# dylkot/cNMF

Measured on NVIDIA H100. Metric: NMF restarts/sec on NxG counts, K-sweep x100 seeds, 1/2/4/8 H100 vs sklearn CPU, higher is better.
Workload: dtype f32 (2-pass split-fp16 tensor-core products of group-normalised factors x exact integer counts, fp32 accumulate)

## Files before the change

cnmf_b200/csrc/gemm_tf32x3.cu:

```cuda
#include <cuda.h>
#include <cuda_runtime.h>
#include <cstdint>
#include <cstdio>
#include <algorithm>
#include <map>
#include <mutex>
#include <tuple>

#include "common.cuh"
#include "gemm.h"

namespace cnmf {

namespace {

constexpr int BM = 128;
constexpr int BN = 128;
constexpr int BK = 32;
constexpr int NUM_THREADS = 384;
constexpr long long WAIT_TIMEOUT_CYCLES = 4000000000LL;

template <int STAGES, bool BEXACT>
struct SmemLayout {
  static constexpr int A_BYTES = BM * BK * 4;
  static constexpr int B_BYTES = BN * BK * 4;
  static constexpr int STAGE_BYTES = 2 * A_BYTES + (BEXACT ? 1 : 2) * B_BYTES;
  static constexpr int BAR_OFFSET = STAGES * STAGE_BYTES;
  static constexpr int TOTAL = BAR_OFFSET + 2 * STAGES * 8;
  static constexpr int DYN_BYTES = TOTAL + 1024;
  static_assert(DYN_BYTES <= 227 * 1024, "pipeline stages do not fit the shared memory of an SM");
};

__device__ __forceinline__ void mbar_init(uint32_t bar, uint32_t count) {
  asm volatile("mbarrier.init.shared::cta.b64 [%0], %1;" ::"r"(bar), "r"(count) : "memory");
}
__device__ __forceinline__ void mbar_arrive_expect_tx(uint32_t bar, uint32_t bytes) {
  asm volatile("mbarrier.arrive.expect_tx.shared::cta.b64 _, [%0], %1;" ::"r"(bar), "r"(bytes) : "memory");
}
__device__ __forceinline__ void mbar_arrive(uint32_t bar) {
  asm volatile("mbarrier.arrive.shared::cta.b64 _, [%0];" ::"r"(bar) : "memory");
}
__device__ __forceinline__ bool mbar_try_wait(uint32_t bar, uint32_t parity) {
  uint32_t ok;
  asm volatile(
      "{\n\t.reg .pred p;\n\t"
      "mbarrier.try_wait.parity.shared::cta.b64 p, [%1], %2;\n\t"
      "selp.u32 %0, 1, 0, p;\n\t}"
      : "=r"(ok)
      : "r"(bar), "r"(parity)
      : "memory");
  return ok != 0;
}
__device__ __forceinline__ void mbar_wait(uint32_t bar, uint32_t parity) {
  if (mbar_try_wait(bar, parity)) return;
  const long long t0 = clock64();
  while (!mbar_try_wait(bar, parity)) {
    if (clock64() - t0 > WAIT_TIMEOUT_CYCLES) __trap();
  }
}
__device__ __forceinline__ void tma_load_2d(uint32_t dst, const CUtensorMap* map, uint32_t bar, int c0, int c1) {
  asm volatile(
      "cp.async.bulk.tensor.2d.shared::cluster.global.mbarrier::complete_tx::bytes [%0], [%1, {%3, %4}], [%2];"
      ::"r"(dst), "l"(reinterpret_cast<uint64_t>(map)), "r"(bar), "r"(c0), "r"(c1)
      : "memory");
}

__device__ __forceinline__ uint64_t make_smem_desc(uint32_t smem_addr) {
  uint64_t d = 0;
  d |= static_cast<uint64_t>((smem_addr & 0x3FFFFu) >> 4);
  d |= static_cast<uint64_t>(1) << 16;
  d |= static_cast<uint64_t>(1024 >> 4) << 32;
  d |= static_cast<uint64_t>(1) << 62;
  return d;
}

__device__ __forceinline__ void named_bar_sync(uint32_t id, uint32_t count) {
  asm volatile("bar.sync %0, %1;" ::"r"(id), "r"(count) : "memory");
}
__device__ __forceinline__ void named_bar_arrive(uint32_t id, uint32_t count) {
  asm volatile("bar.arrive %0, %1;" ::"r"(id), "r"(count) : "memory");
}

__device__ __forceinline__ void wgmma_fence() { asm volatile("wgmma.fence.sync.aligned;" ::: "memory"); }
__device__ __forceinline__ void wgmma_commit() { asm volatile("wgmma.commit_group.sync.aligned;" ::: "memory"); }
template <int N>
__device__ __forceinline__ void wgmma_wait() { asm volatile("wgmma.wait_group.sync.aligned %0;" ::"n"(N) : "memory"); }

template <bool F16>
__device__ __forceinline__ void wgmma_m64n128(float (&d)[64], uint64_t adesc, uint64_t bdesc, uint32_t acc) {
  if constexpr (F16) {
    asm volatile(
      "{\n\t.reg .pred p;\n\t"
      "setp.ne.b32 p, %66, 0;\n\t"
      "wgmma.mma_async.sync.aligned.m64n128k16.f32.f16.f16 {"
      "%0, %1, %2, %3, %4, %5, %6, %7, %8, %9, %10, %11, %12, %13, %14, %15, "
      "%16, %17, %18, %19, %20, %21, %22, %23, %24, %25, %26, %27, %28, %29, %30, %31, "
      "%32, %33, %34, %35, %36, %37, %38, %39, %40, %41, %42, %43, %44, %45, %46, %47, "
      "%48, %49, %50, %51, %52, %53, %54, %55, %56, %57, %58, %59, %60, %61, %62, %63 "
      "}, %64, %65, p, 1, 1, 0, 0;\n\t}"
      : "+f"(d[0]), "+f"(d[1]), "+f"(d[2]), "+f"(d[3]), "+f"(d[4]), "+f"(d[5]), "+f"(d[6]), "+f"(d[7]),
        "+f"(d[8]), "+f"(d[9]), "+f"(d[10]), "+f"(d[11]), "+f"(d[12]), "+f"(d[13]), "+f"(d[14]), "+f"(d[15]),
        "+f"(d[16]), "+f"(d[17]), "+f"(d[18]), "+f"(d[19]), "+f"(d[20]), "+f"(d[21]), "+f"(d[22]), "+f"(d[23]),
        "+f"(d[24]), "+f"(d[25]), "+f"(d[26]), "+f"(d[27]), "+f"(d[28]), "+f"(d[29]), "+f"(d[30]), "+f"(d[31]),
        "+f"(d[32]), "+f"(d[33]), "+f"(d[34]), "+f"(d[35]), "+f"(d[36]), "+f"(d[37]), "+f"(d[38]), "+f"(d[39]),
        "+f"(d[40]), "+f"(d[41]), "+f"(d[42]), "+f"(d[43]), "+f"(d[44]), "+f"(d[45]), "+f"(d[46]), "+f"(d[47]),
        "+f"(d[48]), "+f"(d[49]), "+f"(d[50]), "+f"(d[51]), "+f"(d[52]), "+f"(d[53]), "+f"(d[54]), "+f"(d[55]),
        "+f"(d[56]), "+f"(d[57]), "+f"(d[58]), "+f"(d[59]), "+f"(d[60]), "+f"(d[61]), "+f"(d[62]), "+f"(d[63])
      : "l"(adesc), "l"(bdesc), "r"(acc));
  } else {
    asm volatile(
      "{\n\t.reg .pred p;\n\t"
      "setp.ne.b32 p, %66, 0;\n\t"
      "wgmma.mma_async.sync.aligned.m64n128k8.f32.tf32.tf32 {"
      "%0, %1, %2, %3, %4, %5, %6, %7, %8, %9, %10, %11, %12, %13, %14, %15, "
      "%16, %17, %18, %19, %20, %21, %22, %23, %24, %25, %26, %27, %28, %29, %30, %31, "
      "%32, %33, %34, %35, %36, %37, %38, %39, %40, %41, %42, %43, %44, %45, %46, %47, "
      "%48, %49, %50, %51, %52, %53, %54, %55, %56, %57, %58, %59, %60, %61, %62, %63 "
      "}, %64, %65, p, 1, 1;\n\t}"
      : "+f"(d[0]), "+f"(d[1]), "+f"(d[2]), "+f"(d[3]), "+f"(d[4]), "+f"(d[5]), "+f"(d[6]), "+f"(d[7]),
        "+f"(d[8]), "+f"(d[9]), "+f"(d[10]), "+f"(d[11]), "+f"(d[12]), "+f"(d[13]), "+f"(d[14]), "+f"(d[15]),
        "+f"(d[16]), "+f"(d[17]), "+f"(d[18]), "+f"(d[19]), "+f"(d[20]), "+f"(d[21]), "+f"(d[22]), "+f"(d[23]),
        "+f"(d[24]), "+f"(d[25]), "+f"(d[26]), "+f"(d[27]), "+f"(d[28]), "+f"(d[29]), "+f"(d[30]), "+f"(d[31]),
        "+f"(d[32]), "+f"(d[33]), "+f"(d[34]), "+f"(d[35]), "+f"(d[36]), "+f"(d[37]), "+f"(d[38]), "+f"(d[39]),
        "+f"(d[40]), "+f"(d[41]), "+f"(d[42]), "+f"(d[43]), "+f"(d[44]), "+f"(d[45]), "+f"(d[46]), "+f"(d[47]),
        "+f"(d[48]), "+f"(d[49]), "+f"(d[50]), "+f"(d[51]), "+f"(d[52]), "+f"(d[53]), "+f"(d[54]), "+f"(d[55]),
        "+f"(d[56]), "+f"(d[57]), "+f"(d[58]), "+f"(d[59]), "+f"(d[60]), "+f"(d[61]), "+f"(d[62]), "+f"(d[63])
      : "l"(adesc), "l"(bdesc), "r"(acc));
  }
}

struct TileOrder {
  int m_tiles, n_tiles, group, group_n;
};

__host__ __device__ __forceinline__ void decode_item(int w, const TileOrder& o, int& mt, int& nt, int& z) {
  const int per_slice = o.m_tiles * o.n_tiles;
  z = w / per_slice;
  int r = w - z * per_slice;
  const int q_tiles = o.group_n ? o.n_tiles : o.m_tiles;
  const int p_tiles = o.group_n ? o.m_tiles : o.n_tiles;
  const int g0 = r / (o.group * p_tiles) * o.group;
  r -= g0 * p_tiles;
  const int gq = q_tiles - g0 < o.group ? q_tiles - g0 : o.group;
  const int p = r / gq, q = g0 + r % gq;
  mt = o.group_n ? p : q;
  nt = o.group_n ? q : p;
}

template <int STAGES, bool BEXACT, bool F16>
__device__ __forceinline__ void
gemm_body(const CUtensorMap& tmA_hi, const CUtensorMap& tmA_lo, const CUtensorMap& tmB_hi, const CUtensorMap& tmB_lo,
          float* __restrict__ C, int M, int ldc, long long c_split_stride,
          const TileOrder& ord, int splits, int total_kb, int kb_per_split, int chain_kb,
          const float* __restrict__ out_scale, const float* __restrict__ a_tile_scale, int a_tiles, int a_gshift) {
  static_assert(!F16 || BEXACT, "the fp16 path exists for exact integer B operands only");
  constexpr int BKE = F16 ? 2 * BK : BK;
  constexpr int KSTEP_BYTES = 32;
  using L = SmemLayout<STAGES, BEXACT>;
  extern __shared__ uint8_t smem_raw[];
  const uint32_t smem_base = (smem_u32(smem_raw) + 1023u) & ~1023u;

  const uint32_t bar_base = smem_base + L::BAR_OFFSET;
  auto full_bar = [&](int s) { return bar_base + 8u * s; };
  auto empty_bar = [&](int s) { return bar_base + 8u * (STAGES + s); };

  const int wg = threadIdx.x >> 7;
  const int warp = (threadIdx.x >> 5) & 3;
  const int lane = threadIdx.x & 31;

  if (threadIdx.x == 0) {
    for (int s = 0; s < STAGES; ++s) {
      mbar_init(full_bar(s), 1);
      mbar_init(empty_bar(s), 8);
    }
    asm volatile("fence.mbarrier_init.release.cluster;" ::: "memory");
  }
  __syncthreads();

  const int items = ord.m_tiles * ord.n_tiles * splits;

  if (wg == 0) {
    if (threadIdx.x == 0) {
      int stage = 0;
      uint32_t phase = 0;
      constexpr uint32_t stage_tx = static_cast<uint32_t>(L::STAGE_BYTES);
      for (int w = blockIdx.x; w < items; w += gridDim.x) {
        int mt, nt, z;
        decode_item(w, ord, mt, nt, z);
        const int kb0 = z * kb_per_split;
        const int kb1 = min(total_kb, kb0 + kb_per_split);
        for (int kb = kb0; kb < kb1; ++kb) {
          mbar_wait(empty_bar(stage), phase ^ 1u);
          const uint32_t st = smem_base + stage * L::STAGE_BYTES;
          mbar_arrive_expect_tx(full_bar(stage), stage_tx);
          tma_load_2d(st, &tmA_hi, full_bar(stage), kb * BKE, mt * BM);
          tma_load_2d(st + L::A_BYTES, &tmA_lo, full_bar(stage), kb * BKE, mt * BM);
          tma_load_2d(st + 2 * L::A_BYTES, &tmB_hi, full_bar(stage), kb * BKE, nt * BN);
          if constexpr (!BEXACT) tma_load_2d(st + 2 * L::A_BYTES + L::B_BYTES, &tmB_lo, full_bar(stage), kb * BKE, nt * BN);
          if (++stage == STAGES) { stage = 0; phase ^= 1u; }
        }
      }
    }
  } else {
    constexpr uint32_t TURN_BAR = 1, TURN_THREADS = 256;
    const int cw = wg - 1;
    const uint32_t a_off = static_cast<uint32_t>(cw * 64 * 128);
    if (cw == 1) named_bar_arrive(TURN_BAR, TURN_THREADS);
    int stage = 0;
    uint32_t phase = 0;
    for (int w = blockIdx.x; w < items; w += gridDim.x) {
      int mt, nt, z;
      decode_item(w, ord, mt, nt, z);
      const int kb0 = z * kb_per_split;
      const int kb1 = min(total_kb, kb0 + kb_per_split);
      const int row0 = mt * BM + cw * 64 + warp * 16 + (lane >> 2);
      float acc[64];
#pragma unroll
      for (int i = 0; i < 64; ++i) acc[i] = 0.f;
      const float* sc_row0 = (F16 && a_tile_scale && row0 < M) ? a_tile_scale + static_cast<long long>(row0) * a_tiles : nullptr;
      const float* sc_row1 = (F16 && a_tile_scale && row0 + 8 < M) ? a_tile_scale + static_cast<long long>(row0 + 8) * a_tiles : nullptr;
      for (int c0 = kb0; c0 < kb1; c0 += chain_kb) {
        const int c1 = min(kb1, c0 + chain_kb);
        float d[64];
        int prev = -1;
        for (int kb = c0; kb < c1; ++kb) {
          mbar_wait(full_bar(stage), phase);
          named_bar_sync(TURN_BAR + cw, TURN_THREADS);
          const uint32_t st = smem_base + stage * L::STAGE_BYTES;
          const uint64_t a_hi = make_smem_desc(st + a_off);
          const uint64_t a_lo = make_smem_desc(st + L::A_BYTES + a_off);
          const uint64_t b_hi = make_smem_desc(st + 2 * L::A_BYTES);
          const uint64_t b_lo = make_smem_desc(st + 2 * L::A_BYTES + L::B_BYTES);
          wgmma_fence();
#pragma unroll
          for (int k = 0; k < BK * 4 / KSTEP_BYTES; ++k) {
            const uint64_t koff = static_cast<uint64_t>((k * KSTEP_BYTES) >> 4);
            const uint32_t acc0 = (kb > c0 || k > 0) ? 1u : 0u;
            wgmma_m64n128<F16>(d, a_lo + koff, b_hi + koff, acc0);
            if constexpr (!BEXACT) wgmma_m64n128<F16>(d, a_hi + koff, b_lo + koff, 1u);
            wgmma_m64n128<F16>(d, a_hi + koff, b_hi + koff, 1u);
          }
          wgmma_commit();
          named_bar_arrive(TURN_BAR + (cw ^ 1), TURN_THREADS);
          if (prev >= 0) {
            wgmma_wait<1>();
            if (lane == 0) mbar_arrive(empty_bar(prev));
          }
          prev = stage;
          if (++stage == STAGES) { stage = 0; phase ^= 1u; }
        }
        wgmma_wait<0>();
        if (lane == 0) mbar_arrive(empty_bar(prev));
        if constexpr (F16) {
          const float s0 = sc_row0 ? sc_row0[c0 >> a_gshift] : 1.f;
          const float s1 = sc_row1 ? sc_row1[c0 >> a_gshift] : 1.f;
#pragma unroll
          for (int i = 0; i < 64; i += 4) {
            acc[i] = fmaf(d[i], s0, acc[i]);
            acc[i + 1] = fmaf(d[i + 1], s0, acc[i + 1]);
            acc[i + 2] = fmaf(d[i + 2], s1, acc[i + 2]);
            acc[i + 3] = fmaf(d[i + 3], s1, acc[i + 3]);
          }
        } else {
#pragma unroll
          for (int i = 0; i < 64; ++i) acc[i] += d[i];
        }
      }
      constexpr int EPI_J = 8;
      float* cbase = C + static_cast<long long>(z) * c_split_stride;
      const int colq = nt * BN + 2 * (lane & 3);
#pragma unroll
      for (int j0 = 0; j0 < 16; j0 += EPI_J) {
        float2 sc[EPI_J];
#pragma unroll
        for (int j = 0; j < EPI_J; ++j) {
          const int col = colq + 8 * (j0 + j);
          sc[j] = out_scale && col < ldc ? *reinterpret_cast<const float2*>(out_scale + col) : make_float2(1.f, 1.f);
        }
#pragma unroll
        for (int j = 0; j < EPI_J; ++j) {
          const int col = colq + 8 * (j0 + j);
          if (col >= ldc) continue;
          const float* a = acc + 4 * (j0 + j);
          if (row0 < M)
            *reinterpret_cast<float2*>(cbase + static_cast<long long>(row0) * ldc + col) =
                make_float2(a[0] * sc[j].x, a[1] * sc[j].y);
          if (row0 + 8 < M)
            *reinterpret_cast<float2*>(cbase + static_cast<long long>(row0 + 8) * ldc + col) =
                make_float2(a[2] * sc[j].x, a[3] * sc[j].y);
        }
      }
    }
    if (cw == 0) named_bar_sync(TURN_BAR, TURN_THREADS);
  }
}

template <int STAGES, bool BEXACT, bool F16>
__global__ void __launch_bounds__(NUM_THREADS, 1)
gemm_tf32x3_kernel(const __grid_constant__ CUtensorMap tmA_hi, const __grid_constant__ CUtensorMap tmA_lo,
                   const __grid_constant__ CUtensorMap tmB_hi, const __grid_constant__ CUtensorMap tmB_lo,
                   float* __restrict__ C, int M, int ldc, long long c_split_stride,
                   const TileOrder ord, int splits, int total_kb, int kb_per_split, int chain_kb,
                   const float* __restrict__ out_scale, const float* __restrict__ a_tile_scale, int a_tiles, int a_gshift) {
  gemm_body<STAGES, BEXACT, F16>(tmA_hi, tmA_lo, tmB_hi, tmB_lo, C, M, ldc, c_split_stride, ord, splits, total_kb,
                                 kb_per_split, chain_kb, out_scale, a_tile_scale, a_tiles, a_gshift);
}

typedef CUresult (*PFN_encodeTiled)(CUtensorMap*, CUtensorMapDataType, cuuint32_t, void*, const cuuint64_t*,
                                    const cuuint64_t*, const cuuint32_t*, const cuuint32_t*, CUtensorMapInterleave,
                                    CUtensorMapSwizzle, CUtensorMapL2promotion, CUtensorMapFloatOOBfill);

PFN_encodeTiled get_encode_fn() {
  static PFN_encodeTiled fn = nullptr;
  static std::once_flag once;
  std::call_once(once, [] {
    void* p = nullptr;
    cudaDriverEntryPointQueryResult qres;
    if (cudaGetDriverEntryPoint("cuTensorMapEncodeTiled", &p, cudaEnableDefault, &qres) == cudaSuccess &&
        qres == cudaDriverEntryPointSuccess)
      fn = reinterpret_cast<PFN_encodeTiled>(p);
  });
  return fn;
}

struct MapKey {
  const void* ptr; int rows, cols, ld, box_rows, f16;
  bool operator<(const MapKey& o) const {
    return std::tie(ptr, rows, cols, ld, box_rows, f16) < std::tie(o.ptr, o.rows, o.cols, o.ld, o.box_rows, o.f16);
  }
};

int make_map(CUtensorMap* map, const float* ptr, int rows, int cols, int ld, int box_rows, bool f16 = false) {
  static std::mutex mu;
  static std::map<MapKey, CUtensorMap> cache;
  const MapKey key{ptr, rows, cols, ld, box_rows, f16 ? 1 : 0};
  {
    std::lock_guard<std::mutex> lock(mu);
    auto it = cache.find(key);
    if (it != cache.end()) { *map = it->second; return 0; }
  }
  PFN_encodeTiled enc = get_encode_fn();
  if (!enc) { set_last_error("cuTensorMapEncodeTiled entry point not available"); return -2; }
  const int esize = f16 ? 2 : 4;
  cuuint64_t dims[2] = {static_cast<cuuint64_t>(cols), static_cast<cuuint64_t>(rows)};
  cuuint64_t strides[1] = {static_cast<cuuint64_t>(ld) * esize};
  cuuint32_t box[2] = {static_cast<cuuint32_t>(128 / esize), static_cast<cuuint32_t>(box_rows)};
  cuuint32_t estr[2] = {1, 1};
  CUresult r = enc(map, f16 ? CU_TENSOR_MAP_DATA_TYPE_FLOAT16 : CU_TENSOR_MAP_DATA_TYPE_FLOAT32, 2, const_cast<float*>(ptr), dims, strides, box, estr,
                   CU_TENSOR_MAP_INTERLEAVE_NONE, CU_TENSOR_MAP_SWIZZLE_128B, CU_TENSOR_MAP_L2_PROMOTION_L2_256B,
                   CU_TENSOR_MAP_FLOAT_OOB_FILL_NONE);
  if (r != CUDA_SUCCESS) {
    set_last_error("cuTensorMapEncodeTiled failed with CUresult " + std::to_string(static_cast<int>(r)));
    return -2;
  }
  std::lock_guard<std::mutex> lock(mu);
  if (cache.size() >= 512) cache.clear();
  cache.emplace(key, *map);
  return 0;
}

static double order_bytes(int q_tiles, int p_tiles, double q_panel, double p_panel, int group, int grid, double budget) {
  const long long waves = (static_cast<long long>(group) * p_tiles + grid - 1) / grid;
  const double q_reads = group * q_panel <= budget ? 1.0 : static_cast<double>(std::min<long long>(p_tiles, waves));
  return q_tiles * q_panel * q_reads + static_cast<double>((q_tiles + group - 1) / group) * p_tiles * p_panel;
}

static TileOrder pick_tile_order(int m_tiles, int n_tiles, double a_panel, double b_panel, int grid, long long l2_bytes) {
  const double budget = 0.5 * static_cast<double>(l2_bytes);
  TileOrder best{m_tiles, n_tiles, m_tiles, 0};
  double best_bytes = order_bytes(m_tiles, n_tiles, a_panel, b_panel, m_tiles, grid, budget);
  for (int gn = 0; gn < 2; ++gn) {
    const int q = gn ? n_tiles : m_tiles, p = gn ? m_tiles : n_tiles;
    const double qb = gn ? b_panel : a_panel, pb = gn ? a_panel : b_panel;
    int prev = 0;
    for (int ng = 1; ng <= q; ++ng) {
      const int g = (q + ng - 1) / ng;
      if (g == prev) continue;
      prev = g;
      const double b = order_bytes(q, p, qb, pb, g, grid, budget);
      if (b < best_bytes) { best_bytes = b; best = TileOrder{m_tiles, n_tiles, g, gn}; }
    }
  }
  return best;
}

template <int STAGES, bool BEXACT, bool F16>
int launch(const GemmArgs& g, cudaStream_t stream) {
  using L = SmemLayout<STAGES, BEXACT>;
  constexpr int BKE = F16 ? 2 * BK : BK;
  CUtensorMap mAh, mAl, mBh, mBl;
  int rc;
  if ((rc = make_map(&mAh, g.A_hi, g.M, g.Kd, g.lda, BM, F16))) return rc;
  if ((rc = make_map(&mAl, g.A_lo, g.M, g.Kd, g.lda, BM, F16))) return rc;
  if ((rc = make_map(&mBh, g.B_hi, g.N, g.Kd, g.ldb, BN, F16))) return rc;
  if ((rc = make_map(&mBl, BEXACT ? g.B_hi : g.B_lo, g.N, g.Kd, g.ldb, BN, F16))) return rc;
  int dev = 0, sms = 0, l2 = 0;
  CNMF_CUDA_CHECK(cudaGetDevice(&dev));
  CNMF_CUDA_CHECK(cudaDeviceGetAttribute(&sms, cudaDevAttrMultiProcessorCount, dev));
  CNMF_CUDA_CHECK(cudaDeviceGetAttribute(&l2, cudaDevAttrL2CacheSize, dev));
  const int m_tiles = (g.M + BM - 1) / BM;
  const int n_tiles = (g.N + BN - 1) / BN;
  const int total_kb = (g.Kd + BKE - 1) / BKE;
  int splits = g.splits < 1 ? 1 : g.splits;
  if (splits > total_kb) splits = total_kb;
  int kb_per_split = (total_kb + splits - 1) / splits;
  if (F16 && (kb_per_split & 1)) ++kb_per_split;
  splits = (total_kb + kb_per_split - 1) / kb_per_split;
  if (splits != g.splits_effective) { set_last_error("gemm: splits_effective mismatch (use gemm_effective_splits)"); return -1; }

  auto kern = gemm_tf32x3_kernel<STAGES, BEXACT, F16>;
  static bool attr_set[64] = {};
  if (dev < 0 || dev >= 64 || !attr_set[dev]) {
    CNMF_CUDA_CHECK(cudaFuncSetAttribute(kern, cudaFuncAttributeMaxDynamicSharedMemorySize, L::DYN_BYTES));
    if (dev >= 0 && dev < 64) attr_set[dev] = true;
  }
  const int items = m_tiles * n_tiles * splits;
  const int grid = items < sms ? items : sms;
  const double kslice_row = static_cast<double>(kb_per_split) * BK * 4;
  const TileOrder ord = pick_tile_order(m_tiles, n_tiles, BM * kslice_row * 2, BN * kslice_row * (BEXACT ? 1 : 2),
                                        grid, l2);
  kern<<<grid, NUM_THREADS, L::DYN_BYTES, stream>>>(mAh, mAl, mBh, mBl, g.C, g.M, g.ldc, g.c_split_stride,
                                                    ord, splits, total_kb, kb_per_split, BEXACT ? 2 : 1,
                                                    g.out_col_scale, g.a_tile_scale, g.a_tiles, 3);
  CNMF_CUDA_CHECK(cudaGetLastError());
  return 0;
}

}

int gemm_fixed_splits(int Kd, int f16) {
  const int bke = f16 ? 2 * BK : BK;
  const int total_kb = (Kd + bke - 1) / bke;
  const int s = std::max(1, std::min(16, (total_kb + 63) / 64));
  return gemm_effective_splits(Kd, s, f16);
}

int gemm_effective_splits(int Kd, int splits, int f16) {
  const int bke = f16 ? 2 * BK : BK;
  const int total_kb = (Kd + bke - 1) / bke;
  if (splits < 1) splits = 1;
  if (splits > total_kb) splits = total_kb;
  int kb_per_split = (total_kb + splits - 1) / splits;
  if (f16 && (kb_per_split & 1)) ++kb_per_split;
  return (total_kb + kb_per_split - 1) / kb_per_split;
}

int gemm_tf32x3(const GemmArgs& g, cudaStream_t stream) {
  CNMF_REQUIRE(g.M > 0 && g.N > 0 && g.Kd > 0, "gemm: empty problem");
  CNMF_REQUIRE(g.lda % 4 == 0 && g.ldb % 4 == 0 && g.ldc % 4 == 0, "gemm: leading dimensions must be multiples of 4 floats");
  CNMF_REQUIRE((reinterpret_cast<uintptr_t>(g.A_hi) | reinterpret_cast<uintptr_t>(g.A_lo) |
                reinterpret_cast<uintptr_t>(g.B_hi) | reinterpret_cast<uintptr_t>(g.B_lo) |
                reinterpret_cast<uintptr_t>(g.C) | reinterpret_cast<uintptr_t>(g.out_col_scale)) % 16 == 0,
               "gemm: pointers must be 16-byte aligned");
  if (g.f16) {
    CNMF_REQUIRE(g.b_exact, "gemm: the fp16 path needs an exact B operand");
    CNMF_REQUIRE(g.lda % 8 == 0 && g.ldb % 8 == 0, "gemm: fp16 leading dimensions must be multiples of 8 halves");
    CNMF_REQUIRE(!g.a_tile_scale || g.a_tiles * 512 >= g.Kd, "gemm: a_tiles does not cover the reduction length");
    return launch<4, true, true>(g, stream);
  }
  if (g.b_exact) return launch<4, true, false>(g, stream);
  return launch<3, false, false>(g, stream);
}

}
```

Measured before the change: 503.9.

## Use 2-CTA clusters with TMA multicast to share A tiles across N-tile pairs

Launches the GEMM as 2-CTA clusters. The two CTAs in a cluster work on adjacent N tiles with the same M tile, and each loads half of the A (hi/lo) tile and multicasts it to both. A per-stage peer-free mbarrier makes a CTA wait until its partner has freed that stage before issuing the multicast. The aim is to halve A-operand traffic from L2/HBM, at the cost of cross-CTA synchronisation, idle work when n_tiles is odd, and grid sizing limited by cluster occupancy.

Measured after the change: 525.4, median of 6. 4.3% higher.

```diff
diff --git a/cnmf_b200/csrc/gemm_tf32x3.cu b/cnmf_b200/csrc/gemm_tf32x3.cu
--- a/cnmf_b200/csrc/gemm_tf32x3.cu
+++ b/cnmf_b200/csrc/gemm_tf32x3.cu
@@ -26,7 +26,7 @@
   static constexpr int B_BYTES = BN * BK * 4;
   static constexpr int STAGE_BYTES = 2 * A_BYTES + (BEXACT ? 1 : 2) * B_BYTES;
   static constexpr int BAR_OFFSET = STAGES * STAGE_BYTES;
-  static constexpr int TOTAL = BAR_OFFSET + 2 * STAGES * 8;
+  static constexpr int TOTAL = BAR_OFFSET + 3 * STAGES * 8;
   static constexpr int DYN_BYTES = TOTAL + 1024;
   static_assert(DYN_BYTES <= 227 * 1024, "pipeline stages do not fit the shared memory of an SM");
 };
@@ -63,6 +63,26 @@
       "cp.async.bulk.tensor.2d.shared::cluster.global.mbarrier::complete_tx::bytes [%0], [%1, {%3, %4}], [%2];"
       ::"r"(dst), "l"(reinterpret_cast<uint64_t>(map)), "r"(bar), "r"(c0), "r"(c1)
       : "memory");
+}
+__device__ __forceinline__ void tma_load_2d_multicast(uint32_t dst, const CUtensorMap* map, uint32_t bar, int c0, int c1,
+                                                      uint16_t mask) {
+  asm volatile(
+      "cp.async.bulk.tensor.2d.shared::cluster.global.mbarrier::complete_tx::bytes.multicast::cluster"
+      " [%0], [%1, {%3, %4}], [%2], %5;"
+      ::"r"(dst), "l"(reinterpret_cast<uint64_t>(map)), "r"(bar), "r"(c0), "r"(c1), "h"(mask)
+      : "memory");
+}
+
+__device__ __forceinline__ void mbar_arrive_remote(uint32_t bar, uint32_t rank) {
+  asm volatile(
+      "{\n\t.reg .b32 remote;\n\t"
+      "mapa.shared::cluster.u32 remote, %0, %1;\n\t"
+      "mbarrier.arrive.shared::cluster.b64 _, [remote];\n\t}"
+      ::"r"(bar), "r"(rank)
+      : "memory");
+}
+__device__ __forceinline__ void cluster_sync() {
+  asm volatile("barrier.cluster.arrive.release;\n\tbarrier.cluster.wait.acquire;" ::: "memory");
 }
 
 __device__ __forceinline__ uint64_t make_smem_desc(uint32_t smem_addr) {
@@ -130,28 +150,28 @@
 }
 
 struct TileOrder {
-  int m_tiles, n_tiles, group, group_n;
+  int m_tiles, n_pairs, group, group_n;
 };
 
-__host__ __device__ __forceinline__ void decode_item(int w, const TileOrder& o, int& mt, int& nt, int& z) {
-  const int per_slice = o.m_tiles * o.n_tiles;
+__host__ __device__ __forceinline__ void decode_item(int w, const TileOrder& o, int& mt, int& np, int& z) {
+  const int per_slice = o.m_tiles * o.n_pairs;
   z = w / per_slice;
   int r = w - z * per_slice;
-  const int q_tiles = o.group_n ? o.n_tiles : o.m_tiles;
-  const int p_tiles = o.group_n ? o.m_tiles : o.n_tiles;
+  const int q_tiles = o.group_n ? o.n_pairs : o.m_tiles;
+  const int p_tiles = o.group_n ? o.m_tiles : o.n_pairs;
   const int g0 = r / (o.group * p_tiles) * o.group;
   r -= g0 * p_tiles;
   const int gq = q_tiles - g0 < o.group ? q_tiles - g0 : o.group;
   const int p = r / gq, q = g0 + r % gq;
   mt = o.group_n ? p : q;
-  nt = o.group_n ? q : p;
+  np = o.group_n ? q : p;
 }
 
 template <int STAGES, bool BEXACT, bool F16>
 __device__ __forceinline__ void
 gemm_body(const CUtensorMap& tmA_hi, const CUtensorMap& tmA_lo, const CUtensorMap& tmB_hi, const CUtensorMap& tmB_lo,
           float* __restrict__ C, int M, int ldc, long long c_split_stride,
-          const TileOrder& ord, int splits, int total_kb, int kb_per_split, int chain_kb,
+          const TileOrder& ord, int n_tiles, int splits, int total_kb, int kb_per_split, int chain_kb,
           const float* __restrict__ out_scale, const float* __restrict__ a_tile_scale, int a_tiles, int a_gshift) {
   static_assert(!F16 || BEXACT, "the fp16 path exists for exact integer B operands only");
   constexpr int BKE = F16 ? 2 * BK : BK;
@@ -163,38 +183,46 @@
   const uint32_t bar_base = smem_base + L::BAR_OFFSET;
   auto full_bar = [&](int s) { return bar_base + 8u * s; };
   auto empty_bar = [&](int s) { return bar_base + 8u * (STAGES + s); };
+  auto peer_free_bar = [&](int s) { return bar_base + 8u * (2 * STAGES + s); };
 
   const int wg = threadIdx.x >> 7;
   const int warp = (threadIdx.x >> 5) & 3;
   const int lane = threadIdx.x & 31;
+  const int rank = blockIdx.x & 1, cluster = blockIdx.x >> 1, clusters = gridDim.x >> 1;
 
   if (threadIdx.x == 0) {
     for (int s = 0; s < STAGES; ++s) {
       mbar_init(full_bar(s), 1);
       mbar_init(empty_bar(s), 8);
+      mbar_init(peer_free_bar(s), 1);
     }
     asm volatile("fence.mbarrier_init.release.cluster;" ::: "memory");
   }
-  __syncthreads();
-
-  const int items = ord.m_tiles * ord.n_tiles * splits;
+  cluster_sync();
+
+  const int items = ord.m_tiles * ord.n_pairs * splits;
 
   if (wg == 0) {
     if (threadIdx.x == 0) {
       int stage = 0;
       uint32_t phase = 0;
       constexpr uint32_t stage_tx = static_cast<uint32_t>(L::STAGE_BYTES);
-      for (int w = blockIdx.x; w < items; w += gridDim.x) {
-        int mt, nt, z;
-        decode_item(w, ord, mt, nt, z);
+      constexpr uint32_t HALF_A = L::A_BYTES / 2;
+      for (int w = cluster; w < items; w += clusters) {
+        int mt, np, z;
+        decode_item(w, ord, mt, np, z);
+        const int nt = 2 * np + rank;
         const int kb0 = z * kb_per_split;
         const int kb1 = min(total_kb, kb0 + kb_per_split);
         for (int kb = kb0; kb < kb1; ++kb) {
           mbar_wait(empty_bar(stage), phase ^ 1u);
+          mbar_arrive_remote(peer_free_bar(stage), rank ^ 1);
+          mbar_wait(peer_free_bar(stage), phase);
           const uint32_t st = smem_base + stage * L::STAGE_BYTES;
           mbar_arrive_expect_tx(full_bar(stage), stage_tx);
-          tma_load_2d(st, &tmA_hi, full_bar(stage), kb * BKE, mt * BM);
-          tma_load_2d(st + L::A_BYTES, &tmA_lo, full_bar(stage), kb * BKE, mt * BM);
+          tma_load_2d_multicast(st + rank * HALF_A, &tmA_hi, full_bar(stage), kb * BKE, mt * BM + rank * (BM / 2), 0x3);
+          tma_load_2d_multicast(st + L::A_BYTES + rank * HALF_A, &tmA_lo, full_bar(stage), kb * BKE,
+                                mt * BM + rank * (BM / 2), 0x3);
           tma_load_2d(st + 2 * L::A_BYTES, &tmB_hi, full_bar(stage), kb * BKE, nt * BN);
           if constexpr (!BEXACT) tma_load_2d(st + 2 * L::A_BYTES + L::B_BYTES, &tmB_lo, full_bar(stage), kb * BKE, nt * BN);
           if (++stage == STAGES) { stage = 0; phase ^= 1u; }
@@ -208,9 +236,10 @@
     if (cw == 1) named_bar_arrive(TURN_BAR, TURN_THREADS);
     int stage = 0;
     uint32_t phase = 0;
-    for (int w = blockIdx.x; w < items; w += gridDim.x) {
-      int mt, nt, z;
-      decode_item(w, ord, mt, nt, z);
+    for (int w = cluster; w < items; w += clusters) {
+      int mt, np, z;
+      decode_item(w, ord, mt, np, z);
+      const int nt = 2 * np + rank;
       const int kb0 = z * kb_per_split;
       const int kb1 = min(total_kb, kb0 + kb_per_split);
       const int row0 = mt * BM + cw * 64 + warp * 16 + (lane >> 2);
@@ -266,6 +295,7 @@
           for (int i = 0; i < 64; ++i) acc[i] += d[i];
         }
       }
+      if (nt >= n_tiles) continue;
       constexpr int EPI_J = 8;
       float* cbase = C + static_cast<long long>(z) * c_split_stride;
       const int colq = nt * BN + 2 * (lane & 3);
@@ -293,17 +323,18 @@
     }
     if (cw == 0) named_bar_sync(TURN_BAR, TURN_THREADS);
   }
+  cluster_sync();
 }
 
 template <int STAGES, bool BEXACT, bool F16>
-__global__ void __launch_bounds__(NUM_THREADS, 1)
+__global__ void __cluster_dims__(2, 1, 1) __launch_bounds__(NUM_THREADS, 1)
 gemm_tf32x3_kernel(const __grid_constant__ CUtensorMap tmA_hi, const __grid_constant__ CUtensorMap tmA_lo,
                    const __grid_constant__ CUtensorMap tmB_hi, const __grid_constant__ CUtensorMap tmB_lo,
                    float* __restrict__ C, int M, int ldc, long long c_split_stride,
-                   const TileOrder ord, int splits, int total_kb, int kb_per_split, int chain_kb,
+                   const TileOrder ord, int n_tiles, int splits, int total_kb, int kb_per_split, int chain_kb,
                    const float* __restrict__ out_scale, const float* __restrict__ a_tile_scale, int a_tiles, int a_gshift) {
-  gemm_body<STAGES, BEXACT, F16>(tmA_hi, tmA_lo, tmB_hi, tmB_lo, C, M, ldc, c_split_stride, ord, splits, total_kb,
-                                 kb_per_split, chain_kb, out_scale, a_tile_scale, a_tiles, a_gshift);
+  gemm_body<STAGES, BEXACT, F16>(tmA_hi, tmA_lo, tmB_hi, tmB_lo, C, M, ldc, c_split_stride, ord, n_tiles, splits,
+                                 total_kb, kb_per_split, chain_kb, out_scale, a_tile_scale, a_tiles, a_gshift);
 }
 
 typedef CUresult (*PFN_encodeTiled)(CUtensorMap*, CUtensorMapDataType, cuuint32_t, void*, const cuuint64_t*,
@@ -365,12 +396,12 @@
   return q_tiles * q_panel * q_reads + static_cast<double>((q_tiles + group - 1) / group) * p_tiles * p_panel;
 }
 
-static TileOrder pick_tile_order(int m_tiles, int n_tiles, double a_panel, double b_panel, int grid, long long l2_bytes) {
+static TileOrder pick_tile_order(int m_tiles, int n_pairs, double a_panel, double b_panel, int grid, long long l2_bytes) {
   const double budget = 0.5 * static_cast<double>(l2_bytes);
-  TileOrder best{m_tiles, n_tiles, m_tiles, 0};
-  double best_bytes = order_bytes(m_tiles, n_tiles, a_panel, b_panel, m_tiles, grid, budget);
+  TileOrder best{m_tiles, n_pairs, m_tiles, 0};
+  double best_bytes = order_bytes(m_tiles, n_pairs, a_panel, b_panel, m_tiles, grid, budget);
   for (int gn = 0; gn < 2; ++gn) {
-    const int q = gn ? n_tiles : m_tiles, p = gn ? m_tiles : n_tiles;
+    const int q = gn ? n_pairs : m_tiles, p = gn ? m_tiles : n_pairs;
     const double qb = gn ? b_panel : a_panel, pb = gn ? a_panel : b_panel;
     int prev = 0;
     for (int ng = 1; ng <= q; ++ng) {
@@ -378,7 +409,7 @@
       if (g == prev) continue;
       prev = g;
       const double b = order_bytes(q, p, qb, pb, g, grid, budget);
-      if (b < best_bytes) { best_bytes = b; best = TileOrder{m_tiles, n_tiles, g, gn}; }
+      if (b < best_bytes) { best_bytes = b; best = TileOrder{m_tiles, n_pairs, g, gn}; }
     }
   }
   return best;
@@ -390,16 +421,16 @@
   constexpr int BKE = F16 ? 2 * BK : BK;
   CUtensorMap mAh, mAl, mBh, mBl;
   int rc;
-  if ((rc = make_map(&mAh, g.A_hi, g.M, g.Kd, g.lda, BM, F16))) return rc;
-  if ((rc = make_map(&mAl, g.A_lo, g.M, g.Kd, g.lda, BM, F16))) return rc;
+  if ((rc = make_map(&mAh, g.A_hi, g.M, g.Kd, g.lda, BM / 2, F16))) return rc;
+  if ((rc = make_map(&mAl, g.A_lo, g.M, g.Kd, g.lda, BM / 2, F16))) return rc;
   if ((rc = make_map(&mBh, g.B_hi, g.N, g.Kd, g.ldb, BN, F16))) return rc;
   if ((rc = make_map(&mBl, BEXACT ? g.B_hi : g.B_lo, g.N, g.Kd, g.ldb, BN, F16))) return rc;
-  int dev = 0, sms = 0, l2 = 0;
+  int dev = 0, l2 = 0;
   CNMF_CUDA_CHECK(cudaGetDevice(&dev));
-  CNMF_CUDA_CHECK(cudaDeviceGetAttribute(&sms, cudaDevAttrMultiProcessorCount, dev));
   CNMF_CUDA_CHECK(cudaDeviceGetAttribute(&l2, cudaDevAttrL2CacheSize, dev));
   const int m_tiles = (g.M + BM - 1) / BM;
   const int n_tiles = (g.N + BN - 1) / BN;
+  const int n_pairs = (n_tiles + 1) / 2;
   const int total_kb = (g.Kd + BKE - 1) / BKE;
   int splits = g.splits < 1 ? 1 : g.splits;
   if (splits > total_kb) splits = total_kb;
@@ -409,18 +440,25 @@
   if (splits != g.splits_effective) { set_last_error("gemm: splits_effective mismatch (use gemm_effective_splits)"); return -1; }
 
   auto kern = gemm_tf32x3_kernel<STAGES, BEXACT, F16>;
-  static bool attr_set[64] = {};
-  if (dev < 0 || dev >= 64 || !attr_set[dev]) {
+  static int max_clusters[64] = {};
+  int clusters_cap = dev >= 0 && dev < 64 ? max_clusters[dev] : 0;
+  if (clusters_cap == 0) {
     CNMF_CUDA_CHECK(cudaFuncSetAttribute(kern, cudaFuncAttributeMaxDynamicSharedMemorySize, L::DYN_BYTES));
-    if (dev >= 0 && dev < 64) attr_set[dev] = true;
-  }
-  const int items = m_tiles * n_tiles * splits;
-  const int grid = items < sms ? items : sms;
+    cudaLaunchConfig_t cfg = {};
+    cfg.gridDim = dim3(2, 1, 1);
+    cfg.blockDim = dim3(NUM_THREADS, 1, 1);
+    cfg.dynamicSmemBytes = L::DYN_BYTES;
+    CNMF_CUDA_CHECK(cudaOccupancyMaxActiveClusters(&clusters_cap, kern, &cfg));
+    if (clusters_cap < 1) { set_last_error("gemm: no 2-CTA cluster of this kernel fits the device"); return -1; }
+    if (dev >= 0 && dev < 64) max_clusters[dev] = clusters_cap;
+  }
+  const int items = m_tiles * n_pairs * splits;
+  const int clusters = items < clusters_cap ? items : clusters_cap;
   const double kslice_row = static_cast<double>(kb_per_split) * BK * 4;
-  const TileOrder ord = pick_tile_order(m_tiles, n_tiles, BM * kslice_row * 2, BN * kslice_row * (BEXACT ? 1 : 2),
-                                        grid, l2);
-  kern<<<grid, NUM_THREADS, L::DYN_BYTES, stream>>>(mAh, mAl, mBh, mBl, g.C, g.M, g.ldc, g.c_split_stride,
-                                                    ord, splits, total_kb, kb_per_split, BEXACT ? 2 : 1,
+  const TileOrder ord = pick_tile_order(m_tiles, n_pairs, BM * kslice_row * 2, 2 * BN * kslice_row * (BEXACT ? 1 : 2),
+                                        clusters, l2);
+  kern<<<2 * clusters, NUM_THREADS, L::DYN_BYTES, stream>>>(mAh, mAl, mBh, mBl, g.C, g.M, g.ldc, g.c_split_stride,
+                                                            ord, n_tiles, splits, total_kb, kb_per_split, BEXACT ? 2 : 1,
                                                     g.out_col_scale, g.a_tile_scale, g.a_tiles, 3);
   CNMF_CUDA_CHECK(cudaGetLastError());
   return 0;
```
